# hamidthri/navbot_ppo

Hardware: AMD Instinct MI355X
Metric: env_steps_per_sec (higher is better)
Workload: dtype f32; 1 GPU; BASELINE configs[1]: 4096 envs/GPU, stage_1 (32 segments), 10 beams, PPO mlp64x2, rollout=512, 50 full-batch epochs, episode cap 500; n_envs_total=4096, n_envs_per_gpu=4096, rollout_len=512, epochs=50, policy=mlp64x2, parallelism=env-shard dp1, update_arith=bf16x3, rollout=persistent kernel (navsim_rollout_mlp64)

## Files before the change

### navbot_ppo_amd/csrc/ppo_mlp64_x3s.h

```cpp
#pragma once

namespace x3s {

typedef unsigned u32x4 __attribute__((ext_vector_type(4)));
typedef unsigned u32x2 __attribute__((ext_vector_type(2)));
typedef short s16x4 __attribute__((ext_vector_type(4)));
typedef float v4f __attribute__((ext_vector_type(4)));

constexpr int SW = 4;
constexpr int kPieceB = 32 * 128;
constexpr int kImgB = 3 * kPieceB;

struct SmemS {
    uint16_t W2p[3][H][H];
    uint16_t W2Tp[3][H][H];
    uint16_t W1p[3][H][16];
    float b1[H], b2[H], w3[H], w4[H];
    unsigned char img[SW][2][kImgB];
};
static_assert(sizeof(SmemS) <= 160 * 1024, "LDS");
static_assert(offsetof(SmemS, img) % 128 == 0 && kImgB % 128 == 0, "image bases keep the low 7 address bits of a lane offset (the XOR swizzles)");
static_assert(sizeof(SmemS::img) >= 4 * ((Layout<16>::P_ACTOR + 6) & ~3) * sizeof(float), "reduction rows fit the images");
static_assert(sizeof(SmemS::img) / SW >= 96 * 64 * sizeof(float), "lane partials fit a wave's images");

#ifndef X3S_GUARD
#define X3S_GUARD ""
#endif
#define X3S_G "s_nop 0\n\t"
#define X3S_MFMA32_V_AV(acc, A, B) asm volatile(X3S_GUARD "v_mfma_f32_32x32x16_bf16 %0, %1, %2, %0" : "+v"(acc) : "a"(A), "v"(B))
#define X3S_MFMA32_V_AA(acc, A, B) asm volatile(X3S_GUARD "v_mfma_f32_32x32x16_bf16 %0, %1, %2, %0" : "+v"(acc) : "a"(A), "a"(B))
#define X3S_MFMA32G_V_AV(acc, A, B) asm volatile(X3S_G "v_mfma_f32_32x32x16_bf16 %0, %1, %2, %0" : "+v"(acc) : "a"(A), "v"(B))
#define X3S_MFMA32G_V_AA(acc, A, B) asm volatile(X3S_G "v_mfma_f32_32x32x16_bf16 %0, %1, %2, %0" : "+v"(acc) : "a"(A), "a"(B))
#define X3S_MFMA32_VZ_AV(acc, A, B) asm volatile(X3S_G "v_mfma_f32_32x32x16_bf16 %0, %1, %2, 0" : "=&v"(acc) : "a"(A), "v"(B))
#define X3S_MFMA32_VZ_AA(acc, A, B) asm volatile(X3S_G "v_mfma_f32_32x32x16_bf16 %0, %1, %2, 0" : "=&v"(acc) : "a"(A), "a"(B))
#define X3S_MFMA32_A_AV(acc, A, B) asm volatile(X3S_GUARD "v_mfma_f32_32x32x16_bf16 %0, %1, %2, %0" : "+a"(acc) : "a"(A), "v"(B))
#define X3S_MFMA32_AZ_AV(acc, A, B) asm volatile(X3S_G "v_mfma_f32_32x32x16_bf16 %0, %1, %2, 0" : "=&a"(acc) : "a"(A), "v"(B))
#define X3S_MFMA32_A_AA(acc, A, B) asm volatile(X3S_GUARD "v_mfma_f32_32x32x16_bf16 %0, %1, %2, %0" : "+a"(acc) : "a"(A), "a"(B))
#define X3S_MFMA16_A_AA(acc, A, B) asm volatile(X3S_GUARD "v_mfma_f32_16x16x32_bf16 %0, %1, %2, %0" : "+a"(acc) : "a"(A), "a"(B))
#define X3S_MFMA16_V_AA(acc, A, B) asm volatile(X3S_GUARD "v_mfma_f32_16x16x32_bf16 %0, %1, %2, %0" : "+v"(acc) : "a"(A), "a"(B))
#define X3S_MFMA16G_V_AA(acc, A, B) asm volatile(X3S_G "v_mfma_f32_16x16x32_bf16 %0, %1, %2, %0" : "+v"(acc) : "a"(A), "a"(B))
#define X3S_MFMA16_A_VA(acc, A, B) asm volatile(X3S_GUARD "v_mfma_f32_16x16x32_bf16 %0, %1, %2, %0" : "+a"(acc) : "v"(A), "a"(B))
#define X3S_MFMA16_V_VA(acc, A, B) asm volatile(X3S_GUARD "v_mfma_f32_16x16x32_bf16 %0, %1, %2, %0" : "+v"(acc) : "v"(A), "a"(B))
#define X3S_MFMA16G_A_AA(acc, A, B) asm volatile(X3S_G "v_mfma_f32_16x16x32_bf16 %0, %1, %2, %0" : "+a"(acc) : "a"(A), "a"(B))
#define X3S_MFMA16_A_AV(acc, A, B) asm volatile(X3S_GUARD "v_mfma_f32_16x16x32_bf16 %0, %1, %2, %0" : "+a"(acc) : "a"(A), "v"(B))

#define X3S_REP10(F, b) F(b + 0); F(b + 1); F(b + 2); F(b + 3); F(b + 4); F(b + 5); F(b + 6); F(b + 7); F(b + 8); F(b + 9);

__device__ __forceinline__ void settle(f32x16& a, f32x16& b) { asm volatile("s_nop 7\n\ts_nop 3" : "+v"(a), "+v"(b)); }

__device__ __forceinline__ void split_a(unsigned& p0, float& ra, float& rb, const float a, const float b) {
    asm volatile("v_cvt_pk_bf16_f32 %0, %3, %4\n\t"
                 "v_lshlrev_b32 %1, 16, %0\n\t"
                 "v_and_b32 %2, 0xffff0000, %0\n\t"
                 "v_sub_f32 %1, %3, %1\n\t"
                 "v_sub_f32 %2, %4, %2"
                 : "=&v"(p0), "=&v"(ra), "=&v"(rb) : "v"(a), "v"(b));
}
__device__ __forceinline__ void split_b(unsigned& p1, unsigned& p2, const float ra, const float rb) {
    float t0, t1;
    asm volatile("v_cvt_pk_bf16_f32 %0, %4, %5\n\t"
                 "v_lshlrev_b32 %2, 16, %0\n\t"
                 "v_and_b32 %3, 0xffff0000, %0\n\t"
                 "v_sub_f32 %2, %4, %2\n\t"
                 "v_sub_f32 %3, %5, %3\n\t"
                 "v_cvt_pk_bf16_f32 %1, %2, %3"
                 : "=&v"(p1), "=&v"(p2), "=&v"(t0), "=&v"(t1) : "v"(ra), "v"(rb));
}
__device__ __forceinline__ void relu4(float (&h)[16], const f32x16& c, const int g) {
    float y0, y1, y2, y3;
    asm volatile("v_max_i32 %0, %4, 0\n\tv_max_i32 %1, %5, 0\n\tv_max_i32 %2, %6, 0\n\tv_max_i32 %3, %7, 0"
                 : "=&v"(y0), "=&v"(y1), "=&v"(y2), "=&v"(y3) : "v"(c[4 * g]), "v"(c[4 * g + 1]), "v"(c[4 * g + 2]), "v"(c[4 * g + 3]));
    h[4 * g] = y0; h[4 * g + 1] = y1; h[4 * g + 2] = y2; h[4 * g + 3] = y3;
}
template <bool ACTOR>
__device__ __forceinline__ void dh2_value(float& h, float& pw3, float& pw4, float& pb2, const float g3, const float g4, const float w3,
                                          const float w4) {
    float d;
    if constexpr (ACTOR)
        asm volatile("v_fmac_f32 %1, %0, %5\n\t"
                     "v_fmac_f32 %2, %0, %6\n\t"
                     "v_mul_f32 %4, %6, %8\n\t"
                     "v_fmac_f32 %4, %5, %7\n\t"
                     "v_cmp_lt_f32 vcc, 0, %0\n\t"
                     "v_cndmask_b32 %0, 0, %4, vcc\n\t"
                     "v_add_f32 %3, %3, %0"
                     : "+v"(h), "+v"(pw3), "+v"(pw4), "+v"(pb2), "=&v"(d) : "v"(g3), "v"(g4), "v"(w3), "v"(w4) : "vcc");
    else
        asm volatile("v_fmac_f32 %1, %0, %4\n\t"
                     "v_mul_f32 %3, %4, %5\n\t"
                     "v_cmp_lt_f32 vcc, 0, %0\n\t"
                     "v_cndmask_b32 %0, 0, %3, vcc\n\t"
                     "v_add_f32 %2, %2, %0"
                     : "+v"(h), "+v"(pw3), "+v"(pb2), "=&v"(d) : "v"(g3), "v"(w3) : "vcc");
}

__device__ __forceinline__ void mask4(float& y0, float& y1, float& y2, float& y3, const float x0, const float x1, const float x2,
                                      const float x3, const unsigned w0, const unsigned w1) {
    asm volatile("v_cmp_ne_u16 vcc, 0, %8\n\t"
                 "v_cndmask_b32 %0, 0, %4, vcc\n\t"
                 "v_cmp_lt_u32 vcc, 0xffff, %8\n\t"
                 "v_cndmask_b32 %1, 0, %5, vcc\n\t"
                 "v_cmp_ne_u16 vcc, 0, %9\n\t"
                 "v_cndmask_b32 %2, 0, %6, vcc\n\t"
                 "v_cmp_lt_u32 vcc, 0xffff, %9\n\t"
                 "v_cndmask_b32 %3, 0, %7, vcc"
                 : "=&v"(y0), "=&v"(y1), "=&v"(y2), "=&v"(y3) : "v"(x0), "v"(x1), "v"(x2), "v"(x3), "v"(w0), "v"(w1) : "vcc");
}

struct P3 {
    u32x4 p[3];
};

__device__ __forceinline__ int fswz(const int m) { return (m & 3) | ((((m >> 2) ^ (m >> 3)) & 1) << 2) | ((((m >> 1) ^ (m >> 3)) & 1) << 3); }

typedef __attribute__((address_space(3))) s16x4* lds_s16x4;
__device__ __forceinline__ u32x2 tr_read(const unsigned char* p) {
    const s16x4 v = __builtin_amdgcn_ds_read_tr16_b64_v4i16((lds_s16x4)p);
    u32x2 r;
    __builtin_memcpy(&r, &v, 8);
    return r;
}
__device__ __forceinline__ u32x4 cat(const u32x2 lo, const u32x2 hi) { return u32x4{lo.x, lo.y, hi.x, hi.y}; }

template <bool ACTOR>
__device__ __forceinline__ void pass_body(SmemS& sm, const float* __restrict__ params, const unsigned char* __restrict__ prep,
                                          const float* __restrict__ act, const float* __restrict__ logp_old,
                                          const float* __restrict__ rtg, const float* __restrict__ adv, long long M, float var,
                                          float clip, float inv_n, float* __restrict__ partial, float* __restrict__ stats_partial) {
    using L = Layout<16>;
    constexpr int OFF_W1 = L::OFF_W1, OFF_B1 = L::OFF_B1, OFF_W2 = L::OFF_W2, OFF_B2 = L::OFF_B2, OFF_W3 = L::OFF_W3, OFF_B3 = L::OFF_B3,
                  OFF_W4 = L::OFF_W4, OFF_B4 = L::OFF_B4;
    constexpr int P = ACTOR ? L::P_ACTOR : L::P_CRITIC;
    constexpr int NT = 64 * SW, kTileBytes = XPad<16>::kTileBytes, kRowsBytes = XPad<16>::kRowsBytes;
    const int tid = threadIdx.x, lane = tid & 63, wave = __builtin_amdgcn_readfirstlane(tid >> 6);
    const int l31 = lane & 31, lhi = lane >> 5, l15 = lane & 15, kk = lane >> 4;

    for (int k = tid; k < H * H / 2; k += NT) {
        const int r = (2 * k) / H, c = (2 * k) % H;
        uint32_t p0, p1, p2;
        bf16x3::split_pair(params[OFF_W2 + r * H + c], params[OFF_W2 + r * H + c + 1], p0, p1, p2);
        const uint32_t pc[3] = {p0, p1, p2};
#pragma unroll
        for (int i = 0; i < 3; ++i) {
            *reinterpret_cast<uint32_t*>(&sm.W2p[i][0][0] + wslot(r, kpos(c))) = pc[i];
            (&sm.W2Tp[i][0][0])[wslot(c, kpos(r))] = (uint16_t)(pc[i] & 0xffffu);
            (&sm.W2Tp[i][0][0])[wslot(c + 1, kpos(r))] = (uint16_t)(pc[i] >> 16);
        }
    }
    for (int k = tid; k < H * 16 / 2; k += NT) {
        const int r = (2 * k) / 16, c = (2 * k) % 16;
        uint32_t p0, p1, p2;
        bf16x3::split_pair(params[OFF_W1 + r * 16 + c], params[OFF_W1 + r * 16 + c + 1], p0, p1, p2);
        *reinterpret_cast<uint32_t*>(&sm.W1p[0][r][c]) = p0;
        *reinterpret_cast<uint32_t*>(&sm.W1p[1][r][c]) = p1;
        *reinterpret_cast<uint32_t*>(&sm.W1p[2][r][c]) = p2;
    }
    if (tid < H) {
        sm.b1[tid] = params[OFF_B1 + tid];
        sm.b2[tid] = params[OFF_B2 + tid];
        sm.w3[tid] = params[OFF_W3 + tid];
        sm.w4[tid] = ACTOR ? params[OFF_W4 + tid] : 0.f;
    }
    const float b3 = params[OFF_B3];
    const float b4 = ACTOR ? params[OFF_B4] : 0.f;
    __syncthreads();

    unsigned char* const smb = reinterpret_cast<unsigned char*>(&sm);
    const int img0 = (int)offsetof(SmemS, img) + wave * 2 * kImgB;
    constexpr int IMG_H = 0, IMG_D = kImgB;
    const int st_base = img0 + l31 * 128 + ((fswz(l31) ^ lhi) << 3);
    auto st_off = [&](const int t, const int j, const int b) { return st_base ^ ((8 * t + 4 * j + 2 * b) << 3); };
    const int g_row = 8 * lhi + (l15 >> 2), g_quad = 4 * ((lane >> 4) & 1) + (lane & 3);
    const int g_base0 = img0 + g_row * 128 + ((g_quad ^ fswz(g_row)) << 3), g_base1 = img0 + (g_row + 4) * 128 + ((g_quad ^ fswz(g_row + 4)) << 3);
    auto g_off = [&](const int t, const int s, const int rd) { return ((rd ? g_base1 : g_base0) ^ (t << 6)) + s * 2048; };
    const int h_row = 8 * kk + (l15 >> 2), h_quad = lane & 3;
    const int h_base0 = img0 + h_row * 128 + ((h_quad ^ fswz(h_row)) << 3), h_base1 = img0 + (h_row + 4) * 128 + ((h_quad ^ fswz(h_row + 4)) << 3);
    auto ldw = [&](const uint16_t* base, const int tt, const int s, const int i) {
        return *reinterpret_cast<const u32x4*>(base + i * H * H + wslot(32 * tt + l31, 16 * s + 8 * lhi));
    };
    const int vec_off = 4 * lhi;
    auto ldv = [&](const float* v, const int t, const int g) { return *reinterpret_cast<const v4f*>(v + 32 * t + 8 * g + vec_off); };

    f32x16 aW2[2][2];
    v4f aW1[4], aB1[4];
#pragma unroll
    for (int a = 0; a < 2; ++a)
#pragma unroll
        for (int b = 0; b < 2; ++b) aW2[a][b] = zero16();
#pragma unroll
    for (int u = 0; u < 4; ++u) aW1[u] = aB1[u] = v4f{0.f, 0.f, 0.f, 0.f};
    float pb2[2][16], pw3[2][16], pw4[2][16];
#pragma unroll
    for (int t = 0; t < 2; ++t)
#pragma unroll
        for (int r = 0; r < 16; ++r) pb2[t][r] = pw3[t][r] = pw4[t][r] = 0.f;
    float adb3 = 0.f, adb4 = 0.f, st0 = 0.f, st1 = 0.f, st2 = 0.f, st3 = 0.f;
    auto keep_w2 = [&]() { asm volatile("" : "+a"(aW2[0][0]), "+a"(aW2[0][1]), "+a"(aW2[1][0]), "+a"(aW2[1][1])); };
    u32x4 ones = {0x3f803f80u, 0x3f803f80u, 0x3f803f80u, 0x3f803f80u};
    asm volatile("" : "+a"(ones));

    const long long n_tiles = (M + 31) / 32;
    const long long gw = (long long)blockIdx.x * SW + wave, stride = (long long)gridDim.x * SW;
    u32x4 xp[3], xbn[3];
    float pre_a0 = 0.f, pre_a1 = 0.f, pre_lp = 0.f, pre_t = 0.f;
    auto request_rows = [&](const long long t) {
        const unsigned char* r = prep + (size_t)t * kTileBytes + ((l31 * 3) * 16 + 8 * lhi) * 2;
        asm volatile("global_load_dwordx4 %0, %3, off\n\tglobal_load_dwordx4 %1, %3, off offset:32\n\tglobal_load_dwordx4 %2, %3, off offset:64"
                     : "=a"(xp[0]), "=a"(xp[1]), "=a"(xp[2]) : "v"(r));
    };
    auto request_cols = [&](const long long t) {
        const unsigned char* c = prep + (size_t)t * kTileBytes + kRowsBytes + (l15 * 32 + 8 * kk) * 2;
        asm volatile("global_load_dwordx4 %0, %3, off\n\tglobal_load_dwordx4 %1, %3, off offset:1024\n\tglobal_load_dwordx4 %2, %3, off offset:2048"
                     : "=a"(xbn[0]), "=a"(xbn[1]), "=a"(xbn[2]) : "v"(c));
    };
    auto request_scalars = [&](const long long t) {
        const long long m = t * 32 + l31;
        if (m < M) {
            if (ACTOR) {
                const float2 a = reinterpret_cast<const float2*>(act)[m];
                pre_a0 = a.x;
                pre_a1 = a.y;
                pre_lp = logp_old[m];
                pre_t = adv[m];
            } else {
                pre_t = rtg[m];
            }
        }
    };
    auto landed = [&]() {
        asm volatile("s_waitcnt vmcnt(0)" : "+a"(xp[0]), "+a"(xp[1]), "+a"(xp[2]), "+a"(xbn[0]), "+a"(xbn[1]), "+a"(xbn[2]));
    };
    static_assert(kTileBytes == 6144 && kRowsBytes == 3072, "offsets of the asm loads: pieces 32 bytes apart in a row, 1024 in the columns");

    struct G1Ops {
        P3 da[4];
    };
    auto g1_gather_pair = [&](G1Ops& o, const int q, const int hb0, const int hb1) {
        const int u = q / 3, i = q % 3;
        o.da[u].p[i] = cat(tr_read(smb + (hb0 ^ (u << 5)) + IMG_D + i * kPieceB), tr_read(smb + (hb1 ^ (u << 5)) + IMG_D + i * kPieceB));
    };
    auto g1_step = [&](const int k, const G1Ops& o, const u32x4 (&xb)[3], const bool guard = false) {
        const int t1 = k / 18, q = k % 18, u = 2 * t1 + (q & 1), e = q >> 1;
        constexpr int kind[9] = {0, 1, 0, 0, 1, 0, 0, 1, 0};
        constexpr int ai[9] = {2, 2, 1, 0, 1, 1, 0, 0, 0};
        constexpr int bi[9] = {0, 0, 1, 2, 0, 0, 1, 0, 0};
        if (guard) {
            if (kind[e]) { X3S_MFMA16G_V_AA(aB1[u], o.da[u].p[ai[e]], ones); }
            else { X3S_MFMA16G_A_AA(aW1[u], o.da[u].p[ai[e]], xb[bi[e]]); }
        } else {
            if (ACTOR) {
                if (kind[e]) { X3S_MFMA16_V_AA(aB1[u], o.da[u].p[ai[e]], ones); }
                else { X3S_MFMA16_A_AA(aW1[u], o.da[u].p[ai[e]], xb[bi[e]]); }
            } else {
                if (kind[e]) { X3S_MFMA16_V_VA(aB1[u], o.da[u].p[ai[e]], ones); }
                else { X3S_MFMA16_A_VA(aW1[u], o.da[u].p[ai[e]], xb[bi[e]]); }
            }
        }
    };
    auto store_pieces = [&](const int img, const int t, const int j, const P3& q) {
#pragma unroll
        for (int i = 0; i < 3; ++i) {
            *reinterpret_cast<u32x2*>(smb + st_off(t, j, 0) + img + i * kPieceB) = u32x2{q.p[i].x, q.p[i].y};
            *reinterpret_cast<u32x2*>(smb + st_off(t, j, 1) + img + i * kPieceB) = u32x2{q.p[i].z, q.p[i].w};
        }
    };
    struct SplitState {
        float ra[4], rb[4];
    };
    auto split_block = [&](const float (&c)[16], const int j, const int b, P3& q, SplitState& ss) {
        const int pr = b >> 1;
        if ((b & 1) == 0) {
            unsigned p0;
            split_a(p0, ss.ra[pr], ss.rb[pr], c[8 * j + 2 * pr], c[8 * j + 2 * pr + 1]);
            q.p[0][pr] = p0;
        } else {
            unsigned p1, p2;
            split_b(p1, p2, ss.ra[pr], ss.rb[pr]);
            q.p[1][pr] = p1;
            q.p[2][pr] = p2;
        }
    };

    f32x16 c1[2], c2[2];
    float h1[2][16];
    P3 hb[4];
    u32x4 wn[2][3], wa[2][3];
    SplitState ss1;
    auto g2_step = [&](const int k, const P3 (&dA)[2][2], const P3 (&hB)[2][2], f32x16 (&aW2)[2][2]) {
        const int t2 = k / 24, sk = (k / 12) & 1, e = (k % 12) >> 1, t1 = k & 1;
        constexpr int ai[6] = {2, 1, 0, 1, 0, 0}, bi[6] = {0, 1, 2, 0, 1, 0};
        X3S_MFMA32_A_AA(aW2[t2][t1], dA[t2][sk].p[ai[e]], hB[t1][sk].p[bi[e]]);
    };
    auto b1_to_c1 = [&](const int q) {
        const v4f b = ldv(sm.b1, q >> 2, q & 3);
        c1[q >> 2][4 * (q & 3)] = b.x; c1[q >> 2][4 * (q & 3) + 1] = b.y; c1[q >> 2][4 * (q & 3) + 2] = b.z; c1[q >> 2][4 * (q & 3) + 3] = b.w;
    };
    auto b2_to_c2 = [&](const int q) {
        const v4f b = ldv(sm.b2, q >> 2, q & 3);
        c2[q >> 2][4 * (q & 3)] = b.x; c2[q >> 2][4 * (q & 3) + 1] = b.y; c2[q >> 2][4 * (q & 3) + 2] = b.z; c2[q >> 2][4 * (q & 3) + 3] = b.w;
    };
    auto ld_wa = [&](const int t, const int i) { wa[t][i] = *reinterpret_cast<const u32x4*>(&sm.W1p[i][32 * t + l31][8 * lhi]); };
    auto ld_wn = [&](const int t, const int i) { wn[t][i] = ldw(&sm.W2p[0][0][0], t, 0, i); };
    auto f1_mfma = [&](const int j) {
        const int t = j / 6, e = j % 6;
        constexpr int wi[6] = {2, 1, 0, 1, 0, 0}, xi[6] = {0, 1, 2, 0, 1, 0};
        if (e == 0) { X3S_MFMA32G_V_AA(c1[t], wa[t][wi[e]], xp[xi[e]]); } else { X3S_MFMA32_V_AA(c1[t], wa[t][wi[e]], xp[xi[e]]); }
    };
    auto ahead_work = [&](const int n, const bool alone) {
        if (n == 11 || n == 13) ld_wa(0, (n - 11) / 2);
        if (n == 15 || n == 17) ld_wa(1, (n - 15) / 2);
        if (n == 19) { ld_wa(0, 2); ld_wa(1, 2); }
        if (n >= 22 && n <= 29) b1_to_c1(n - 22);
        if (n == 42) { ld_wn(0, 0); ld_wn(1, 0); ld_wn(0, 1); ld_wn(1, 1); }
        if (n == 43) {
            ld_wn(0, 2); ld_wn(1, 2);
            if (alone) asm volatile("s_nop 7" : "+v"(c1[0]));
            relu4(h1[0], c1[0], 0);
        }
        if (n == 44) relu4(h1[0], c1[0], 1);
        if (n >= 45 && n <= 52) { split_block(h1[0], 0, n - 45, hb[0], ss1); b2_to_c2(n - 45); }
        if (n == 53) relu4(h1[0], c1[0], 2);
        if (n == 54) relu4(h1[0], c1[0], 3);
        if (n >= 55 && n <= 58) relu4(h1[1], c1[1], n - 55);
    };

    for (int k = lane; k < kImgB / 16; k += 64) reinterpret_cast<u32x4*>(smb + img0 + IMG_D)[k] = u32x4{0u, 0u, 0u, 0u};
    bool have_prev = false;
    if (gw < n_tiles) {
        request_rows(gw);
        request_cols(gw);
        request_scalars(gw);
        auto slot = [&](const int n) {
            if (n == 36) landed();
            if (n >= 36 && n < 48) f1_mfma(n - 36);
            ahead_work(n, true);
        };
        X3S_REP10(slot, 10) X3S_REP10(slot, 20) X3S_REP10(slot, 30) X3S_REP10(slot, 40) X3S_REP10(slot, 50)
    }
    for (long long tile = gw; tile < n_tiles; tile += stride) {
        const bool valid = tile * 32 + l31 < M;
        const float cur_a0 = pre_a0, cur_a1 = pre_a1, cur_lp = pre_lp, cur_t = pre_t;
        const long long tile1 = tile + stride < n_tiles ? tile + stride : tile;

        G1Ops g1o;
        {
            u32x4 wk[4][2];
            SplitState ss;
#pragma unroll
            for (int s = 0; s < 4; ++s) {
                u32x4 w[2][3];
#pragma unroll
                for (int i = 0; i < 3; ++i) { w[0][i] = wn[0][i]; w[1][i] = wn[1][i]; }
                keep_w2();
                auto filler = [&](const int slot) {
                    if (s < 3 && slot >= 1 && slot <= 8) split_block(h1[(s + 1) >> 1], (s + 1) & 1, slot - 1, hb[s + 1], ss);
                    if (s == 3 && slot < 8) wk[slot >> 1][slot & 1] = ldw(&sm.W2p[0][0][0], slot & 1, slot >> 1, 0);
                    if (s < 3 && (slot == 0 || slot == 4 || slot == 9)) {
                        const int i = slot == 0 ? 0 : slot == 4 ? 1 : 2;
                        wn[0][i] = ldw(&sm.W2p[0][0][0], 0, s + 1, i);
                        wn[1][i] = ldw(&sm.W2p[0][0][0], 1, s + 1, i);
                    }
                    if (slot == 9) store_pieces(IMG_H, s >> 1, s & 1, hb[s]);
                };
                if (s == 0) { X3S_MFMA32G_V_AV(c2[0], w[0][2], hb[s].p[0]); } else { X3S_MFMA32_V_AV(c2[0], w[0][2], hb[s].p[0]); }
                filler(0);
                if (s == 0) { X3S_MFMA32G_V_AV(c2[1], w[1][2], hb[s].p[0]); } else { X3S_MFMA32_V_AV(c2[1], w[1][2], hb[s].p[0]); }
                filler(1);
                X3S_MFMA32_V_AV(c2[0], w[0][1], hb[s].p[1]); filler(2);
                X3S_MFMA32_V_AV(c2[1], w[1][1], hb[s].p[1]); filler(3);
                X3S_MFMA32_V_AV(c2[0], w[0][0], hb[s].p[2]); filler(4);
                X3S_MFMA32_V_AV(c2[1], w[1][0], hb[s].p[2]); filler(5);
                X3S_MFMA32_V_AV(c2[0], w[0][1], hb[s].p[0]); filler(6);
                X3S_MFMA32_V_AV(c2[1], w[1][1], hb[s].p[0]); filler(7);
                X3S_MFMA32_V_AV(c2[0], w[0][0], hb[s].p[1]); filler(8);
                X3S_MFMA32_V_AV(c2[1], w[1][0], hb[s].p[1]); filler(9);
            }
            int hb0 = h_base0, hb1 = h_base1;
            asm volatile("" : "+v"(hb0), "+v"(hb1));
            int gq = 0;
#pragma unroll
            for (int s = 0; s < 4; ++s) {
                X3S_MFMA32_V_AV(c2[0], wk[s][0], hb[s].p[0]);
                g1_gather_pair(g1o, gq++, hb0, hb1); g1_gather_pair(g1o, gq++, hb0, hb1);
                X3S_MFMA32_V_AV(c2[1], wk[s][1], hb[s].p[0]);
                g1_gather_pair(g1o, gq++, hb0, hb1);
            }
        }
        settle(c2[0], c2[1]);

        int g1k = 0;
        keep_w2();
        float h2[2][16];
#pragma unroll
        for (int q = 0; q < 8; ++q) {
            g1_step(g1k++, g1o, xbn);
            relu4(h2[q >> 2], c2[q >> 2], q & 3);
        }
        float g3 = 0.f, g4 = 0.f;
        {
            float z3 = 0.f, z4 = 0.f;
#pragma unroll
            for (int t = 0; t < 2; ++t)
#pragma unroll
                for (int g = 0; g < 4; ++g) {
                    const v4f w = ldv(sm.w3, t, g);
                    z3 = fmaf(h2[t][4 * g], w.x, z3); z3 = fmaf(h2[t][4 * g + 1], w.y, z3);
                    z3 = fmaf(h2[t][4 * g + 2], w.z, z3); z3 = fmaf(h2[t][4 * g + 3], w.w, z3);
                    if (ACTOR) {
                        const v4f v = ldv(sm.w4, t, g);
                        z4 = fmaf(h2[t][4 * g], v.x, z4); z4 = fmaf(h2[t][4 * g + 1], v.y, z4);
                        z4 = fmaf(h2[t][4 * g + 2], v.z, z4); z4 = fmaf(h2[t][4 * g + 3], v.w, z4);
                    }
                }
            z3 += __shfl_xor(z3, 32, 64);
            if (ACTOR) z4 += __shfl_xor(z4, 32, 64);
            const float own = (lhi == 0) ? 1.f : 0.f;
            if (valid) {
                z3 += b3;
                z4 += b4;
#ifdef MLP64_DEBUG_Z
                if (lhi == 0) {
                    float* const dbg = partial + (size_t)200 * P;
                    dbg[tile * 32 + l31] = z3;
                    if (ACTOR) dbg[M + tile * 32 + l31] = z4;
                }
#endif
                if (ACTOR) {
                    const float mu0 = 1.0f / (1.0f + expf(-z3));
                    const float mu1 = tanhf(z4);
                    const float d0 = cur_a0 - mu0, d1 = cur_a1 - mu1;
                    const float lp = -0.5f * ((d0 * d0 + d1 * d1) / var) - 1.8378770664093453f - logf(var);
                    const float lr = lp - cur_lp;
                    const float ratio = expf(lr);
                    const float A = cur_t;
                    const float s1 = ratio * A;
                    const float rc = fminf(fmaxf(ratio, 1.0f - clip), 1.0f + clip);
                    const float s2 = rc * A;
                    st0 += own * -fminf(s1, s2);
                    st2 += own * ((ratio - 1.0f) - lr);
                    st3 += (fabsf(ratio - 1.0f) > clip) ? own : 0.f;
                    const bool inside = (ratio >= 1.0f - clip) && (ratio <= 1.0f + clip);
                    const float dL_dratio = (inside || s1 < s2) ? -A : 0.f;
                    const float dL_dlp = dL_dratio * ratio * inv_n;
                    g3 = dL_dlp * (d0 / var) * (mu0 * (1.0f - mu0));
                    g4 = dL_dlp * (d1 / var) * (1.0f - mu1 * mu1);
                } else {
                    const float e = z3 - cur_t;
                    st1 += own * (e * e);
                    g3 = 2.0f * e * inv_n;
                }
            }
            adb3 += own * g3;
            adb4 += own * g4;
#ifdef MLP64_DEBUG_Z
            if (valid && lhi == 0) {
                float* const dbg = partial + (size_t)200 * P;
                dbg[2 * M + tile * 32 + l31] = g3;
                if (ACTOR) dbg[3 * M + tile * 32 + l31] = g4;
            }
#endif
        }
        {
            v4f wn3 = ldv(sm.w3, 0, 0), wn4 = ACTOR ? ldv(sm.w4, 0, 0) : v4f{0.f, 0.f, 0.f, 0.f};
#pragma unroll
            for (int q = 0; q < 8; ++q) {
                const int t = q >> 2, g = q & 3;
                const v4f w = wn3, v = wn4;
                if (q < 7) {
                    wn3 = ldv(sm.w3, (q + 1) >> 2, (q + 1) & 3);
                    if (ACTOR) wn4 = ldv(sm.w4, (q + 1) >> 2, (q + 1) & 3);
                }
                const float wv3[4] = {w.x, w.y, w.z, w.w}, wv4[4] = {v.x, v.y, v.z, v.w};
#pragma unroll
                for (int j = 0; j < 4; ++j) {
                    const int r = 4 * g + j;
                    dh2_value<ACTOR>(h2[t][r], pw3[t][r], pw4[t][r], pb2[t][r], g3, g4, wv3[j], wv4[j]);
                    if (g1k < 36 && (j & 1)) g1_step(g1k++, g1o, xbn);
                }
                if (g1k < 36 && (g & 1)) g1_step(g1k++, g1o, xbn);
            }
        }

        f32x16 c3[2];
        P3 hB[2][2], dA[2][2];
        u32x2 mw[8];
        float d1[2][16];
        auto d_mask = [&](const int k) {
            const int t = k >> 2, r0 = 8 * ((k >> 1) & 1) + 4 * (k & 1);
            mask4(d1[t][r0], d1[t][r0 + 1], d1[t][r0 + 2], d1[t][r0 + 3], c3[t][r0], c3[t][r0 + 1], c3[t][r0 + 2], c3[t][r0 + 3], mw[k].x, mw[k].y);
        };
        {
            P3 db[4];
            u32x4 wk[4][2], wt[2][3];
            SplitState ss;
#pragma unroll
            for (int i = 0; i < 3; ++i) {
                wt[0][i] = ldw(&sm.W2Tp[0][0][0], 0, 0, i);
                wt[1][i] = ldw(&sm.W2Tp[0][0][0], 1, 0, i);
            }
#pragma unroll
            for (int b = 0; b < 8; ++b) {
                g1_step(g1k++, g1o, xbn);
                split_block(h2[0], 0, b, db[0], ss);
            }
#pragma unroll
            for (int s = 0; s < 4; ++s) {
                u32x4 w[2][3];
#pragma unroll
                for (int i = 0; i < 3; ++i) { w[0][i] = wt[0][i]; w[1][i] = wt[1][i]; }
                keep_w2();
                auto filler = [&](const int slot) {
                    if (s == 0 && slot == 0) request_cols(tile);
                    if (s == 0 && slot == 1) request_rows(tile1);
                    if (s == 3 && slot == 0) request_scalars(tile1);
                    if (s < 3 && slot >= 1 && slot <= 8) split_block(h2[(s + 1) >> 1], (s + 1) & 1, slot - 1, db[s + 1], ss);
                    if (s == 3 && slot < 8) wk[slot >> 1][slot & 1] = ldw(&sm.W2Tp[0][0][0], slot & 1, slot >> 1, 0);
                    if (slot == 2 || slot == 5 || slot == 8) {
                        const int q = 3 * s + (slot - 2) / 3, t = q / 6, sk = (q / 3) & 1, i = q % 3;
                        hB[t][sk].p[i] = cat(tr_read(smb + g_off(t, sk, 0) + IMG_H + i * kPieceB), tr_read(smb + g_off(t, sk, 1) + IMG_H + i * kPieceB));
                    }
                    if (s == 3 && (slot == 3 || slot == 4 || slot == 6 || slot == 7)) {
                        const int k0 = 2 * (slot - 3 - (slot > 4));
#pragma unroll
                        for (int k = k0; k < k0 + 2; ++k)
                            mw[k] = *reinterpret_cast<const u32x2*>(smb + st_off(k >> 2, (k >> 1) & 1, k & 1) + IMG_H);
                    }
                    if (s < 3 && (slot == 0 || slot == 4 || slot == 9)) {
                        const int i = slot == 0 ? 0 : slot == 4 ? 1 : 2;
                        wt[0][i] = ldw(&sm.W2Tp[0][0][0], 0, s + 1, i);
                        wt[1][i] = ldw(&sm.W2Tp[0][0][0], 1, s + 1, i);
                    }
                    if (slot == 9) store_pieces(IMG_D, s >> 1, s & 1, db[s]);
                };
                if (s == 0) { X3S_MFMA32_VZ_AV(c3[0], w[0][2], db[s].p[0]); } else { X3S_MFMA32_V_AV(c3[0], w[0][2], db[s].p[0]); }
                filler(0);
                if (s == 0) { X3S_MFMA32_VZ_AV(c3[1], w[1][2], db[s].p[0]); } else { X3S_MFMA32_V_AV(c3[1], w[1][2], db[s].p[0]); }
                filler(1);
                X3S_MFMA32_V_AV(c3[0], w[0][1], db[s].p[1]); filler(2);
                X3S_MFMA32_V_AV(c3[1], w[1][1], db[s].p[1]); filler(3);
                X3S_MFMA32_V_AV(c3[0], w[0][0], db[s].p[2]); filler(4);
                X3S_MFMA32_V_AV(c3[1], w[1][0], db[s].p[2]); filler(5);
                X3S_MFMA32_V_AV(c3[0], w[0][1], db[s].p[0]); filler(6);
                X3S_MFMA32_V_AV(c3[1], w[1][1], db[s].p[0]); filler(7);
                X3S_MFMA32_V_AV(c3[0], w[0][0], db[s].p[1]); filler(8);
                X3S_MFMA32_V_AV(c3[1], w[1][0], db[s].p[1]); filler(9);
            }
            int dq = 0;
            auto gather_d = [&]() {
                const int t = dq / 6, sk = (dq / 3) & 1, i = dq % 3;
                dA[t][sk].p[i] = cat(tr_read(smb + g_off(t, sk, 0) + IMG_D + i * kPieceB), tr_read(smb + g_off(t, sk, 1) + IMG_D + i * kPieceB));
                ++dq;
            };
#pragma unroll
            for (int s = 0; s < 4; ++s) {
                X3S_MFMA32_V_AV(c3[0], wk[s][0], db[s].p[0]);
                gather_d(); gather_d();
            }
#pragma unroll
            for (int s = 0; s < 4; ++s) {
                X3S_MFMA32_V_AV(c3[1], wk[s][1], db[s].p[0]);
                if (s < 2) { gather_d(); gather_d(); }
                else d_mask(s - 2);
            }
        }

        {
            P3 eb[4];
            SplitState ss;
            auto d_work = [&](const int n) {
                if (n == 0 || n == 1) d_mask(2 + n);
                if (n == 20 || n == 21) d_mask(4 + n - 20);
                if (n == 31 || n == 32) d_mask(6 + n - 31);
                const int s = n < 11 ? 0 : n < 20 ? 1 : n < 31 ? 2 : 3, n0 = s == 0 ? 2 : s == 1 ? 11 : s == 2 ? 22 : 33;
                if (n >= n0 && n < n0 + 8) split_block(d1[s >> 1], s & 1, n - n0, eb[s], ss);
                if (n == n0 + 8) store_pieces(IMG_D, s >> 1, s & 1, eb[s]);
            };
            auto slot = [&](const int n) {
                if (n == 36) landed();
                if (n < 36) g2_step(n, dA, hB, aW2);
                else if (n < 48) f1_mfma(n - 36);
                else g2_step(n - 12, dA, hB, aW2);
                d_work(n);
                ahead_work(n, false);
            };
            X3S_REP10(slot, 0) X3S_REP10(slot, 10) X3S_REP10(slot, 20) X3S_REP10(slot, 30) X3S_REP10(slot, 40) X3S_REP10(slot, 50)
        }
        have_prev = true;
    }
    if (have_prev) {
        G1Ops g1o;
#pragma unroll
        for (int q = 0; q < 12; ++q) g1_gather_pair(g1o, q, h_base0, h_base1);
#pragma unroll
        for (int k = 0; k < 36; ++k) g1_step(k, g1o, xbn, true);
    }

    __syncthreads();
    float rb2[2], rw3[2], rw4[2];
    {
        float* const scr = reinterpret_cast<float*>(&sm.img[wave][0][0]);
#pragma unroll
        for (int t = 0; t < 2; ++t)
#pragma unroll
            for (int r = 0; r < 16; ++r) {
                scr[(0 * 32 + 16 * t + r) * 64 + lane] = pb2[t][r];
                scr[(1 * 32 + 16 * t + r) * 64 + lane] = pw3[t][r];
                scr[(2 * 32 + 16 * t + r) * 64 + lane] = pw4[t][r];
            }
        __builtin_amdgcn_fence(__ATOMIC_RELEASE, "wavefront");
        __builtin_amdgcn_wave_barrier();
        const int row = l31, hi = (row >> 2) & 1, r = (row & 3) + 4 * (row >> 3), t = lhi;
        float s[3] = {0.f, 0.f, 0.f};
#pragma unroll
        for (int v = 0; v < 3; ++v) {
            const float* src = scr + (v * 32 + 16 * t + r) * 64 + 32 * hi;
#pragma unroll
            for (int m = 0; m < 32; m += 4) {
                const v4f q = *reinterpret_cast<const v4f*>(src + m);
                s[v] += (q.x + q.y) + (q.z + q.w);
            }
        }
        rb2[0] = s[0]; rw3[0] = s[1]; rw4[0] = s[2];
        rb2[1] = rw3[1] = rw4[1] = 0.f;
    }
    __syncthreads();

    constexpr int RP = (P + 3 + 3) & ~3;
    float s3 = adb3, s4 = adb4, sA = ACTOR ? st0 : st1, sB = st2, sC = st3;
#pragma unroll
    for (int o = 32; o >= 1; o >>= 1) {
        s3 += __shfl_xor(s3, o, 64); s4 += __shfl_xor(s4, o, 64);
        sA += __shfl_xor(sA, o, 64); sB += __shfl_xor(sB, o, 64); sC += __shfl_xor(sC, o, 64);
    }
    float* const red0 = reinterpret_cast<float*>(&sm.img[0][0][0]);
    float* const rowp = red0 + wave * RP;
    {
        auto put = [&](int idx, float v) { rowp[idx] = v; };
#pragma unroll
        for (int t2 = 0; t2 < 2; ++t2)
#pragma unroll
            for (int t1 = 0; t1 < 2; ++t1)
#pragma unroll
                for (int r = 0; r < 16; ++r) put(OFF_W2 + (32 * t2 + c_row(r, lane)) * H + 32 * t1 + l31, aW2[t2][t1][r]);
        put(OFF_B2 + 32 * lhi + l31, rb2[0]);
        put(OFF_W3 + 32 * lhi + l31, rw3[0]);
        if (ACTOR) put(OFF_W4 + 32 * lhi + l31, rw4[0]);
#pragma unroll
        for (int u = 0; u < 4; ++u) {
#pragma unroll
            for (int r = 0; r < 4; ++r) put(OFF_W1 + (16 * u + 4 * kk + r) * 16 + l15, aW1[u][r]);
            if (l15 == 0) {
#pragma unroll
                for (int r = 0; r < 4; ++r) put(OFF_B1 + 16 * u + 4 * kk + r, aB1[u][r]);
            }
        }
        if (lane == 0) {
            put(OFF_B3, s3);
            if (ACTOR) put(OFF_B4, s4);
            put(P + 0, sA);
            put(P + 1, sB);
            put(P + 2, sC);
        }
    }
    __syncthreads();
    float* out = partial + (size_t)blockIdx.x * P;
    const float* red = red0;
    for (int k = tid; k < P; k += NT) out[k] = (red[k] + red[RP + k]) + (red[2 * RP + k] + red[3 * RP + k]);
    if (tid < 3) stats_partial[blockIdx.x * 4 + tid] = (red[P + tid] + red[RP + P + tid]) + (red[2 * RP + P + tid] + red[3 * RP + P + tid]);
}

}

__global__ __launch_bounds__(64 * x3s::SW) void mlp64_pass_both_x3s(const float* __restrict__ params, const unsigned char* __restrict__ prep,
                                                                    const float* __restrict__ act, const float* __restrict__ logp_old,
                                                                    const float* __restrict__ rtg, const float* __restrict__ adv,
                                                                    long long M, float var, float clip, float inv_n, int net_mask,
                                                                    float* __restrict__ partial_a, float* __restrict__ stats_partial_a,
                                                                    float* __restrict__ partial_c, float* __restrict__ stats_partial_c) {
    __shared__ __attribute__((aligned(128))) x3s::SmemS sm;
    if (net_mask & 1) x3s::pass_body<true>(sm, params, prep, act, logp_old, rtg, adv, M, var, clip, inv_n, partial_a, stats_partial_a);
    if (net_mask == 3) __syncthreads();
    if (net_mask & 2) x3s::pass_body<false>(sm, params + Layout<16>::P_ACTOR, prep, act, logp_old, rtg, adv, M, var, clip, inv_n, partial_c, stats_partial_c);
}
```

Baseline: 54.69 million env-steps/s.

## Prefetch head weights early, branchless scalar loads, permlane swap reduction in PPO pass

The w3/w4 head-weight rows are now loaded from LDS during the earlier W2 filler slots and kept in registers for both the forward dot product and the backward loop. The forward head dot product moves to inline fmac asm. The cross-half reduction switches from a shuffle to permlane32_swap. Actor scalar loads become branchless with a clamped index, and the critic rtg prefetch moves to the top of the loop with a running pointer. Also adds reordered W2 weight prefetch, a clamp helper, and optional s_memtime timing stamps that compile only under a macro. The aim is to hide LDS latency and cut branches and cross-lane cost, at the price of higher register pressure.

```diff
diff --git a/navbot_ppo_amd/csrc/ppo_mlp64_x3s.h b/navbot_ppo_amd/csrc/ppo_mlp64_x3s.h
--- a/navbot_ppo_amd/csrc/ppo_mlp64_x3s.h
+++ b/navbot_ppo_amd/csrc/ppo_mlp64_x3s.h
@@ -44,6 +44,15 @@
 #define X3S_MFMA16G_A_AA(acc, A, B) asm volatile(X3S_G "v_mfma_f32_16x16x32_bf16 %0, %1, %2, %0" : "+a"(acc) : "a"(A), "a"(B))
 #define X3S_MFMA16_A_AV(acc, A, B) asm volatile(X3S_GUARD "v_mfma_f32_16x16x32_bf16 %0, %1, %2, %0" : "+a"(acc) : "a"(A), "v"(B))
 
+#ifdef X3S_STAMPS
+#define X3S_STAMP(k) asm volatile("s_memtime %0" : "=s"(stamp_t[k]))
+#define X3S_STAMP2(k, a, b) asm volatile("s_memtime %0" : "=s"(stamp_t[k]), "+v"(a), "+v"(b))
+constexpr int kStampRow = 16;
+#else
+#define X3S_STAMP(k)
+#define X3S_STAMP2(k, a, b)
+#endif
+
 #define X3S_REP10(F, b) F(b + 0); F(b + 1); F(b + 2); F(b + 3); F(b + 4); F(b + 5); F(b + 6); F(b + 7); F(b + 8); F(b + 9);
 
 __device__ __forceinline__ void settle(f32x16& a, f32x16& b) { asm volatile("s_nop 7\n\ts_nop 3" : "+v"(a), "+v"(b)); }
@@ -94,6 +103,22 @@
                      : "+v"(h), "+v"(pw3), "+v"(pb2), "=&v"(d) : "v"(g3), "v"(w3) : "vcc");
 }
 
+template <bool ACTOR>
+__device__ __forceinline__ void zdot4(float& z3, float& z4, const float (&h)[16], const int g, const v4f w, const v4f v) {
+    if constexpr (ACTOR)
+        asm volatile("v_fmac_f32 %0, %2, %6\n\tv_fmac_f32 %1, %2, %10\n\t"
+                     "v_fmac_f32 %0, %3, %7\n\tv_fmac_f32 %1, %3, %11\n\t"
+                     "v_fmac_f32 %0, %4, %8\n\tv_fmac_f32 %1, %4, %12\n\t"
+                     "v_fmac_f32 %0, %5, %9\n\tv_fmac_f32 %1, %5, %13"
+                     : "+v"(z3), "+v"(z4)
+                     : "v"(h[4 * g]), "v"(h[4 * g + 1]), "v"(h[4 * g + 2]), "v"(h[4 * g + 3]), "v"(w.x), "v"(w.y), "v"(w.z), "v"(w.w),
+                       "v"(v.x), "v"(v.y), "v"(v.z), "v"(v.w));
+    else
+        asm volatile("v_fmac_f32 %0, %1, %5\n\tv_fmac_f32 %0, %2, %6\n\tv_fmac_f32 %0, %3, %7\n\tv_fmac_f32 %0, %4, %8"
+                     : "+v"(z3)
+                     : "v"(h[4 * g]), "v"(h[4 * g + 1]), "v"(h[4 * g + 2]), "v"(h[4 * g + 3]), "v"(w.x), "v"(w.y), "v"(w.z), "v"(w.w));
+}
+
 __device__ __forceinline__ void mask4(float& y0, float& y1, float& y2, float& y3, const float x0, const float x1, const float x2,
                                       const float x3, const unsigned w0, const unsigned w1) {
     asm volatile("v_cmp_ne_u16 vcc, 0, %8\n\t"
@@ -107,6 +132,18 @@
                  : "=&v"(y0), "=&v"(y1), "=&v"(y2), "=&v"(y3) : "v"(x0), "v"(x1), "v"(x2), "v"(x3), "v"(w0), "v"(w1) : "vcc");
 }
 
+__device__ __forceinline__ float clamp_ratio(const float x, const float lo, const float hi) {
+    float y;
+    asm("v_max_f32 %0, %1, %2\n\tv_min_f32 %0, %0, %3" : "=&v"(y) : "v"(x), "v"(lo), "v"(hi));
+    return y;
+}
+
+__device__ __forceinline__ float other_half(const float x, const int lhi) {
+    const unsigned u = __float_as_uint(x);
+    const auto r = __builtin_amdgcn_permlane32_swap(u, u, false, false);
+    return __uint_as_float(lhi ? r[0] : r[1]);
+}
+
 struct P3 {
     u32x4 p[3];
 };
@@ -126,7 +163,8 @@
 __device__ __forceinline__ void pass_body(SmemS& sm, const float* __restrict__ params, const unsigned char* __restrict__ prep,
                                           const float* __restrict__ act, const float* __restrict__ logp_old,
                                           const float* __restrict__ rtg, const float* __restrict__ adv, long long M, float var,
-                                          float clip, float inv_n, float* __restrict__ partial, float* __restrict__ stats_partial) {
+                                          float clip, float inv_n, float* __restrict__ partial, float* __restrict__ stats_partial,
+                                          float* __restrict__ stamps) {
     using L = Layout<16>;
     constexpr int OFF_W1 = L::OFF_W1, OFF_B1 = L::OFF_B1, OFF_W2 = L::OFF_W2, OFF_B2 = L::OFF_B2, OFF_W3 = L::OFF_W3, OFF_B3 = L::OFF_B3,
                   OFF_W4 = L::OFF_W4, OFF_B4 = L::OFF_B4;
@@ -199,6 +237,7 @@
     u32x4 ones = {0x3f803f80u, 0x3f803f80u, 0x3f803f80u, 0x3f803f80u};
     asm volatile("" : "+a"(ones));
 
+    const float clip_lo = 1.0f - clip, clip_hi = 1.0f + clip;
     const long long n_tiles = (M + 31) / 32;
     const long long gw = (long long)blockIdx.x * SW + wave, stride = (long long)gridDim.x * SW;
     u32x4 xp[3], xbn[3];
@@ -214,18 +253,21 @@
                      : "=a"(xbn[0]), "=a"(xbn[1]), "=a"(xbn[2]) : "v"(c));
     };
     auto request_scalars = [&](const long long t) {
-        const long long m = t * 32 + l31;
-        if (m < M) {
-            if (ACTOR) {
-                const float2 a = reinterpret_cast<const float2*>(act)[m];
-                pre_a0 = a.x;
-                pre_a1 = a.y;
-                pre_lp = logp_old[m];
-                pre_t = adv[m];
-            } else {
-                pre_t = rtg[m];
-            }
-        }
+        if (ACTOR) {
+            const long long m = t * 32 + l31 < M ? t * 32 + l31 : M - 1;
+            const float2 a = reinterpret_cast<const float2*>(act)[m];
+            pre_a0 = a.x;
+            pre_a1 = a.y;
+            pre_lp = logp_old[m];
+            pre_t = adv[m];
+        } else {
+            const long long m = t * 32 + l31;
+            if (m < M) pre_t = rtg[m];
+        }
+    };
+    auto here = [](long long t) {
+        asm volatile("" : "+s"(t));
+        return t;
     };
     auto landed = [&]() {
         asm volatile("s_waitcnt vmcnt(0)" : "+a"(xp[0]), "+a"(xp[1]), "+a"(xp[2]), "+a"(xbn[0]), "+a"(xbn[1]), "+a"(xbn[2]));
@@ -326,6 +368,7 @@
 
     for (int k = lane; k < kImgB / 16; k += 64) reinterpret_cast<u32x4*>(smb + img0 + IMG_D)[k] = u32x4{0u, 0u, 0u, 0u};
     bool have_prev = false;
+    const float* rtg_next = rtg + (gw + stride) * 32 + l31;
     if (gw < n_tiles) {
         request_rows(gw);
         request_cols(gw);
@@ -337,12 +380,31 @@
         };
         X3S_REP10(slot, 10) X3S_REP10(slot, 20) X3S_REP10(slot, 30) X3S_REP10(slot, 40) X3S_REP10(slot, 50)
     }
+#ifdef X3S_STAMPS
+    unsigned long long stamp_t[8], clk0, clk1, rt0, rt1;
+    unsigned stamp_sum[8] = {0u, 0u, 0u, 0u, 0u, 0u, 0u, 0u};
+    asm volatile("s_memtime %0\n\ts_memrealtime %1\n\ts_waitcnt lgkmcnt(0)" : "=s"(clk0), "=s"(rt0));
+#endif
     for (long long tile = gw; tile < n_tiles; tile += stride) {
+        X3S_STAMP(0);
         const bool valid = tile * 32 + l31 < M;
         const float cur_a0 = pre_a0, cur_a1 = pre_a1, cur_lp = pre_lp, cur_t = pre_t;
         const long long tile1 = tile + stride < n_tiles ? tile + stride : tile;
+        if (!ACTOR) {
+            pre_t = *(rtg_next < rtg + M ? rtg_next : rtg + (M - 1));
+            rtg_next += stride * 32;
+        }
 
         G1Ops g1o;
+        v4f zw3[8], zw4[8];
+        auto ld_zrow = [&](const int n) {
+            if (ACTOR) {
+                if (n & 1) zw4[n >> 1] = ldv(sm.w4, n >> 3, (n >> 1) & 3);
+                else zw3[n >> 1] = ldv(sm.w3, n >> 3, (n >> 1) & 3);
+            } else {
+                zw3[n] = ldv(sm.w3, n >> 2, n & 3);
+            }
+        };
         {
             u32x4 wk[4][2];
             SplitState ss;
@@ -355,8 +417,9 @@
                 auto filler = [&](const int slot) {
                     if (s < 3 && slot >= 1 && slot <= 8) split_block(h1[(s + 1) >> 1], (s + 1) & 1, slot - 1, hb[s + 1], ss);
                     if (s == 3 && slot < 8) wk[slot >> 1][slot & 1] = ldw(&sm.W2p[0][0][0], slot & 1, slot >> 1, 0);
+                    if (s == 3 && slot < 8) ld_zrow(slot);
                     if (s < 3 && (slot == 0 || slot == 4 || slot == 9)) {
-                        const int i = slot == 0 ? 0 : slot == 4 ? 1 : 2;
+                        const int i = slot == 0 ? 2 : slot == 4 ? 1 : 0;
                         wn[0][i] = ldw(&sm.W2p[0][0][0], 0, s + 1, i);
                         wn[1][i] = ldw(&sm.W2p[0][0][0], 1, s + 1, i);
                     }
@@ -386,6 +449,7 @@
                 g1_gather_pair(g1o, gq++, hb0, hb1);
             }
         }
+        X3S_STAMP2(1, c2[0], c2[1]);
         settle(c2[0], c2[1]);
 
         int g1k = 0;
@@ -399,21 +463,16 @@
         float g3 = 0.f, g4 = 0.f;
         {
             float z3 = 0.f, z4 = 0.f;
-#pragma unroll
-            for (int t = 0; t < 2; ++t)
-#pragma unroll
-                for (int g = 0; g < 4; ++g) {
-                    const v4f w = ldv(sm.w3, t, g);
-                    z3 = fmaf(h2[t][4 * g], w.x, z3); z3 = fmaf(h2[t][4 * g + 1], w.y, z3);
-                    z3 = fmaf(h2[t][4 * g + 2], w.z, z3); z3 = fmaf(h2[t][4 * g + 3], w.w, z3);
-                    if (ACTOR) {
-                        const v4f v = ldv(sm.w4, t, g);
-                        z4 = fmaf(h2[t][4 * g], v.x, z4); z4 = fmaf(h2[t][4 * g + 1], v.y, z4);
-                        z4 = fmaf(h2[t][4 * g + 2], v.z, z4); z4 = fmaf(h2[t][4 * g + 3], v.w, z4);
-                    }
-                }
-            z3 += __shfl_xor(z3, 32, 64);
-            if (ACTOR) z4 += __shfl_xor(z4, 32, 64);
+            X3S_STAMP2(2, h2[1][14], h2[1][15]);
+            if (ACTOR) {
+#pragma unroll
+                for (int n = 8; n < 16; ++n) ld_zrow(n);
+            }
+#pragma unroll
+            for (int q = 0; q < 8; ++q) zdot4<ACTOR>(z3, z4, h2[q >> 2], q & 3, zw3[q], zw4[q]);
+            X3S_STAMP2(3, z3, z4);
+            z3 += other_half(z3, lhi);
+            if (ACTOR) z4 += other_half(z4, lhi);
             const float own = (lhi == 0) ? 1.f : 0.f;
             if (valid) {
                 z3 += b3;
@@ -434,12 +493,12 @@
                     const float ratio = expf(lr);
                     const float A = cur_t;
                     const float s1 = ratio * A;
-                    const float rc = fminf(fmaxf(ratio, 1.0f - clip), 1.0f + clip);
+                    const float rc = clamp_ratio(ratio, clip_lo, clip_hi);
                     const float s2 = rc * A;
                     st0 += own * -fminf(s1, s2);
                     st2 += own * ((ratio - 1.0f) - lr);
                     st3 += (fabsf(ratio - 1.0f) > clip) ? own : 0.f;
-                    const bool inside = (ratio >= 1.0f - clip) && (ratio <= 1.0f + clip);
+                    const bool inside = (ratio >= clip_lo) && (ratio <= clip_hi);
                     const float dL_dratio = (inside || s1 < s2) ? -A : 0.f;
                     const float dL_dlp = dL_dratio * ratio * inv_n;
                     g3 = dL_dlp * (d0 / var) * (mu0 * (1.0f - mu0));
@@ -460,15 +519,15 @@
             }
 #endif
         }
+        X3S_STAMP2(4, g3, g4);
         {
-            v4f wn3 = ldv(sm.w3, 0, 0), wn4 = ACTOR ? ldv(sm.w4, 0, 0) : v4f{0.f, 0.f, 0.f, 0.f};
 #pragma unroll
             for (int q = 0; q < 8; ++q) {
                 const int t = q >> 2, g = q & 3;
-                const v4f w = wn3, v = wn4;
-                if (q < 7) {
-                    wn3 = ldv(sm.w3, (q + 1) >> 2, (q + 1) & 3);
-                    if (ACTOR) wn4 = ldv(sm.w4, (q + 1) >> 2, (q + 1) & 3);
+                const v4f w = zw3[q], v = ACTOR ? zw4[q] : v4f{0.f, 0.f, 0.f, 0.f};
+                if (q < 6) {
+                    zw3[q + 2] = ldv(sm.w3, (q + 2) >> 2, (q + 2) & 3);
+                    if (ACTOR) zw4[q + 2] = ldv(sm.w4, (q + 2) >> 2, (q + 2) & 3);
                 }
                 const float wv3[4] = {w.x, w.y, w.z, w.w}, wv4[4] = {v.x, v.y, v.z, v.w};
 #pragma unroll
@@ -503,6 +562,7 @@
                 g1_step(g1k++, g1o, xbn);
                 split_block(h2[0], 0, b, db[0], ss);
             }
+            X3S_STAMP(5);
 #pragma unroll
             for (int s = 0; s < 4; ++s) {
                 u32x4 w[2][3];
@@ -510,9 +570,9 @@
                 for (int i = 0; i < 3; ++i) { w[0][i] = wt[0][i]; w[1][i] = wt[1][i]; }
                 keep_w2();
                 auto filler = [&](const int slot) {
-                    if (s == 0 && slot == 0) request_cols(tile);
-                    if (s == 0 && slot == 1) request_rows(tile1);
-                    if (s == 3 && slot == 0) request_scalars(tile1);
+                    if (s == 0 && slot == 0) request_cols(here(tile));
+                    if (s == 0 && slot == 1) request_rows(here(tile1));
+                    if (ACTOR && s == 3 && slot == 0) request_scalars(here(tile1));
                     if (s < 3 && slot >= 1 && slot <= 8) split_block(h2[(s + 1) >> 1], (s + 1) & 1, slot - 1, db[s + 1], ss);
                     if (s == 3 && slot < 8) wk[slot >> 1][slot & 1] = ldw(&sm.W2Tp[0][0][0], slot & 1, slot >> 1, 0);
                     if (slot == 2 || slot == 5 || slot == 8) {
@@ -526,7 +586,7 @@
                             mw[k] = *reinterpret_cast<const u32x2*>(smb + st_off(k >> 2, (k >> 1) & 1, k & 1) + IMG_H);
                     }
                     if (s < 3 && (slot == 0 || slot == 4 || slot == 9)) {
-                        const int i = slot == 0 ? 0 : slot == 4 ? 1 : 2;
+                        const int i = slot == 0 ? 2 : slot == 4 ? 1 : 0;
                         wt[0][i] = ldw(&sm.W2Tp[0][0][0], 0, s + 1, i);
                         wt[1][i] = ldw(&sm.W2Tp[0][0][0], 1, s + 1, i);
                     }
@@ -564,6 +624,7 @@
             }
         }
 
+        X3S_STAMP(6);
         {
             P3 eb[4];
             SplitState ss;
@@ -586,7 +647,25 @@
             X3S_REP10(slot, 0) X3S_REP10(slot, 10) X3S_REP10(slot, 20) X3S_REP10(slot, 30) X3S_REP10(slot, 40) X3S_REP10(slot, 50)
         }
         have_prev = true;
-    }
+#ifdef X3S_STAMPS
+        asm volatile("s_memtime %0\n\ts_waitcnt lgkmcnt(0)"
+                     : "=s"(stamp_t[7]), "+s"(stamp_t[0]), "+s"(stamp_t[1]), "+s"(stamp_t[2]), "+s"(stamp_t[3]), "+s"(stamp_t[4]), "+s"(stamp_t[5]),
+                       "+s"(stamp_t[6]));
+#pragma unroll
+        for (int k = 0; k < 7; ++k) stamp_sum[k] += (unsigned)(stamp_t[k + 1] - stamp_t[k]);
+        stamp_sum[7] += 1u;
+#endif
+    }
+#ifdef X3S_STAMPS
+    asm volatile("s_memtime %0\n\ts_memrealtime %1\n\ts_waitcnt lgkmcnt(0)" : "=s"(clk1), "=s"(rt1));
+    if (tid == 0) {
+        float* const o = stamps + ((size_t)blockIdx.x * 2 + (ACTOR ? 0 : 1)) * kStampRow;
+#pragma unroll
+        for (int k = 0; k < 8; ++k) o[k] = (float)stamp_sum[k];
+        o[8] = (float)(clk1 - clk0);
+        o[9] = (float)(rt1 - rt0);
+    }
+#endif
     if (have_prev) {
         G1Ops g1o;
 #pragma unroll
@@ -678,7 +757,12 @@
                                                                     float* __restrict__ partial_a, float* __restrict__ stats_partial_a,
                                                                     float* __restrict__ partial_c, float* __restrict__ stats_partial_c) {
     __shared__ __attribute__((aligned(128))) x3s::SmemS sm;
-    if (net_mask & 1) x3s::pass_body<true>(sm, params, prep, act, logp_old, rtg, adv, M, var, clip, inv_n, partial_a, stats_partial_a);
+    float* stamps = nullptr;
+#ifdef X3S_STAMPS
+    stamps = partial_c + (size_t)kWMaxBlocks * Layout<16>::P_CRITIC + 1024;
+    static_assert(1024 + kWMaxBlocks * 2 * x3s::kStampRow <= kWMaxBlocks * (Layout<16>::P_ACTOR - Layout<16>::P_CRITIC), "the stamps fit the free tail");
+#endif
+    if (net_mask & 1) x3s::pass_body<true>(sm, params, prep, act, logp_old, rtg, adv, M, var, clip, inv_n, partial_a, stats_partial_a, stamps);
     if (net_mask == 3) __syncthreads();
-    if (net_mask & 2) x3s::pass_body<false>(sm, params + Layout<16>::P_ACTOR, prep, act, logp_old, rtg, adv, M, var, clip, inv_n, partial_c, stats_partial_c);
-}
+    if (net_mask & 2) x3s::pass_body<false>(sm, params + Layout<16>::P_ACTOR, prep, act, logp_old, rtg, adv, M, var, clip, inv_n, partial_c, stats_partial_c, stamps);
+}
```

Measured after the change: 54.91 million env-steps/s, median of 6. No clear change (+0.4%).
